# VITA-Group/Open-L2O

Measured on AMD Instinct MI355X. Metric: unroll-steps/sec (batch x params x T), L2O-DM on Quadratic d=128, higher is better.
Workload: dtype f32

## Files before the change

open_l2o_amd/csrc/l2o_lstm_bx3.h:

```cpp
#pragma once
#include <type_traits>
#include "l2o_common.h"

namespace l2o {
namespace bx {

typedef unsigned u32x4 __attribute__((ext_vector_type(4)));
typedef float f32x2 __attribute__((ext_vector_type(2)));
typedef __bf16 bf16x2 __attribute__((ext_vector_type(2)));
typedef __bf16 bf16x8 __attribute__((ext_vector_type(8)));

constexpr int kChL1H = 0, kChL2A = 1, kChL2B = 2, kChL1X = 3;
constexpr int kFragWords = 256;
constexpr int kPack = 4;
constexpr int kProducts = 6;
__host__ __device__ constexpr bool packed_default(int pre) { return pre != L2O_PRE_FC_ELU; }
__host__ __device__ constexpr int frags(bool pk) { return pk ? kPack : 3; }
__host__ __device__ constexpr int chunk_mfmas(bool pk) { return (pk ? kPack : kProducts) * kNT; }

__host__ __device__ constexpr int nchunks(int pre) { return pre == L2O_PRE_FC_ELU ? 4 : 3; }
__host__ __device__ constexpr int base(int pre) { return wp_rows(pre) * 64; }
__host__ __device__ constexpr int packed_words(int pre) { return nchunks(pre) * kNT * kPack * kFragWords; }
__host__ __device__ constexpr int level_words(int pre) { return nchunks(pre) * kNT * 3 * kFragWords; }
__host__ __device__ constexpr int frag_off(int pre, bool pk, int ch, int t, int j) {
// ... 176 lines not shown
        w.win1[t] = *reinterpret_cast<const f32x4*>(wp + win_off(PRE) + (kNT + t) * 256 + lane * 4);
    }
    w.wl[t] = p[(wp_row_wl(PRE) + t) * 64];
    if (PRE == L2O_PRE_FC_ELU) {
      w.fcw0[t] = p[(wp_row_fc(PRE) + t) * 64];
      w.fcw1[t] = p[(wp_row_fc(PRE) + kNT + t) * 64];
      w.fcb[t] = p[(wp_row_fc(PRE) + 2 * kNT + t) * 64];
    }
  }
  w.bl = p[wp_row_bl(PRE) * 64];
}

__device__ __forceinline__ f32x4 mfma_bf(u32x4 a, u32x4 b, f32x4 c) {
#ifdef L2O_ABLATE_MFMA
  c[0] = __builtin_fmaf(__uint_as_float(a[0]), __uint_as_float(b[0]), c[0]);
  return c;
#endif
  return __builtin_amdgcn_mfma_f32_16x16x32_bf16(__builtin_bit_cast(bf16x8, a), __builtin_bit_cast(bf16x8, b), c, 0,
                                                  0, 0);
}

template <int LAYER, class W, bool PIN = true>
__device__ __forceinline__ void preload_bias(const W& w, f32x4 (&acc)[kNT]) {
#pragma unroll
  for (int t = 0; t < kNT; ++t) acc[t] = w.bias[(LAYER * kNT + t) * 4];
  if constexpr (PIN) {
#pragma unroll
    for (int t = 0; t < kNT; ++t) asm volatile("" : "+v"(acc[t]));
  }
}

template <int PRE, int CH, int LO, int HI, bool ZERO, bool PK, class W>
__device__ __forceinline__ void issue_pipelined(const W& w, const BOp<PK>& b, f32x4 (&acc)[kNT]) {
  static_assert(PK && W::kLdsFrags, "issue_pipelined: the packed LDS-resident fragments");
  constexpr int DEP = W::kFragDepth;
  u32x4 f[DEP];
  static_for<0, DEP>([&](auto ic) {
    constexpr int i = decltype(ic)::value;
    if constexpr (LO + i < HI) {
      constexpr int n = LO + i;
      f[i] = w.lfr[((CH * kNT + n % kNT) * kPack + n / kNT) * 64];
    }
  });
  __builtin_amdgcn_sched_group_barrier(0x100, (HI - LO) < DEP ? (HI - LO) : DEP, 0);
  static_for<LO, HI>([&](auto nc) {
    constexpr int n = decltype(nc)::value;
    constexpr int p = n / kNT, t = n % kNT, slot = (n - LO) % DEP;
    acc[t] = mfma_bf(f[slot], b.m[p], acc[t]);
    if constexpr (n + DEP < HI) {
      constexpr int m = n + DEP;
      f[slot] = w.lfr[((CH * kNT + m % kNT) * kPack + m / kNT) * 64];
    }
    __builtin_amdgcn_sched_group_barrier(0x008, 1, 0);
    __builtin_amdgcn_sched_group_barrier(0x100, 1, 0);
  });
}

template <int PRE, int CH, int LO, int HI, bool ZERO, bool PK, class W>
__device__ __forceinline__ void issue(const W& w, const BOp<PK>& b, f32x4 (&acc)[kNT]) {
  if constexpr (W::kLdsFrags && W::kFragDepth > 0) {
    issue_pipelined<PRE, CH, LO, HI, ZERO, PK, W>(w, b, acc);
    return;
  }
  static_for<LO, HI>([&](auto nc) {
    constexpr int n = decltype(nc)::value;
    constexpr int p = n / kNT, t = n % kNT;
    if constexpr (W::kLdsFrags) {
      static_assert(PK, "LDS-resident fragments: the packed form");
#ifdef L2O_LDS_ABL_NOFRAG
      acc[t] = mfma_bf(b.m[(p + 1) % kPack], b.m[p], acc[t]);
#else
      acc[t] = mfma_bf(w.lfr[((CH * kNT + t) * kPack + p) * 64], b.m[p], acc[t]);
#endif
      if constexpr (W::kFragFence > 0) {
        if ((n - LO) % W::kFragFence == W::kFragFence - 1) __builtin_amdgcn_sched_barrier(0);
      }
    } else if constexpr (PK) acc[t] = mfma_bf(w.a[CH][t][p], b.m[p], acc[t]);
    else if constexpr (CH == W::kLdsChunk) acc[t] = mfma_bf(w.lch[(t * 3 + prod_w(p)) * 64], b.m[prod_x(p)], acc[t]);
    else acc[t] = mfma_bf(w.a[CH][t][prod_w(p)], b.m[prod_x(p)], acc[t]);
  });
}

template <int T0>
__device__ __forceinline__ void gates_pair(const f32x4 (&acc)[kNT], float (&c)[kNT], float (&h)[kNT]) {
  constexpr int T1 = T0 + 1;
  constexpr float k2 = 2.0f * 1.4426950408889634f;
  const f32x2 one = mk2(1.0f, 1.0f);
  const f32x2 e_i = mk2(fast_exp2(acc[T0][0]), fast_exp2(acc[T1][0]));
  const f32x2 E_j = mk2(fast_exp2(-__builtin_fabsf(acc[T0][1])), fast_exp2(-__builtin_fabsf(acc[T1][1])));
  const f32x2 e_f = mk2(fast_exp2(acc[T0][2]), fast_exp2(acc[T1][2]));
  const f32x2 e_o = mk2(fast_exp2(acc[T0][3]), fast_exp2(acc[T1][3]));
  const f32x2 dij = (one + e_i) * (one + E_j);
  const f32x2 df = one + e_f;
  const f32x2 ij = mk2(fast_rcp(dij.x), fast_rcp(dij.y));
  const f32x2 rf = mk2(fast_rcp(df.x), fast_rcp(df.y));
  f32x2 tj = (one - E_j) * ij;
  tj = mk2(__builtin_copysignf(tj.x, acc[T0][1]), __builtin_copysignf(tj.y, acc[T1][1]));
  const f32x2 cn = __builtin_elementwise_fma(rf, mk2(c[T0], c[T1]), tj);
  const f32x2 ca = cn * mk2(k2, k2);
  const f32x2 E_c = mk2(fast_exp2(-__builtin_fabsf(ca.x)), fast_exp2(-__builtin_fabsf(ca.y)));
  const f32x2 dro = (one + E_c) * (one + e_o);
  const f32x2 ro = mk2(fast_rcp(dro.x), fast_rcp(dro.y));
  const f32x2 hh = (one - E_c) * ro;
  c[T0] = cn.x; c[T1] = cn.y;
  h[T0] = __builtin_copysignf(hh.x, cn.x);
  h[T1] = __builtin_copysignf(hh.y, cn.y);
}

__device__ __forceinline__ void gates5(const f32x4 (&acc)[kNT], float (&c)[kNT], float (&h)[kNT]) {
#ifdef L2O_ABLATE_TRANS
#pragma unroll
  for (int t = 0; t < kNT; ++t) {
    c[t] = (acc[t][2] * 0.25f + 0.75f) * c[t] + (acc[t][0] * 0.25f + 0.5f) * (acc[t][1] * 0.5f);
    h[t] = (c[t] * 0.5f) * (acc[t][3] * 0.25f + 0.5f);
  }
  return;
#endif
#ifdef L2O_ABLATE_GATES
#pragma unroll
  for (int t = 0; t < kNT; ++t) { c[t] = acc[t][2] + acc[t][0]; h[t] = acc[t][1] + acc[t][3]; }
  return;
#endif
  gates_pair<0>(acc, c, h);
  gates_pair<2>(acc, c, h);
  constexpr float k2 = 2.0f * 1.4426950408889634f;
  const float e_i = fast_exp2(acc[4][0]), E_j = fast_exp2(-__builtin_fabsf(acc[4][1]));
  const float e_f = fast_exp2(acc[4][2]), e_o = fast_exp2(acc[4][3]);
  const float ij = fast_rcp((1.0f + e_i) * (1.0f + E_j)), rf = fast_rcp(1.0f + e_f);
  const float cn = __builtin_fmaf(rf, c[4], __builtin_copysignf((1.0f - E_j) * ij, acc[4][1]));
  const float E_c = fast_exp2(-__builtin_fabsf(cn * k2));
  const float ro = fast_rcp((1.0f + E_c) * (1.0f + e_o));
  c[4] = cn;
  h[4] = __builtin_copysignf((1.0f - E_c) * ro, cn);
}

__device__ __forceinline__ void gates5_scalar(const f32x4 (&acc)[kNT], float (&c)[kNT], float (&h)[kNT]) {
  constexpr float k2 = 2.0f * 1.4426950408889634f;
  float e_i[kNT], E_j[kNT], e_f[kNT], e_o[kNT], ij[kNT], rf[kNT], cn[kNT], E_c[kNT], ro[kNT];
#pragma unroll
  for (int t = 0; t < kNT; ++t) e_i[t] = fast_exp2(acc[t][0]);
#pragma unroll
  for (int t = 0; t < kNT; ++t) E_j[t] = fast_exp2(-__builtin_fabsf(acc[t][1]));
#pragma unroll
  for (int t = 0; t < kNT; ++t) e_f[t] = fast_exp2(acc[t][2]);
#pragma unroll
  for (int t = 0; t < kNT; ++t) e_o[t] = fast_exp2(acc[t][3]);
#pragma unroll
  for (int t = 0; t < kNT; ++t) ij[t] = fast_rcp((1.0f + e_i[t]) * (1.0f + E_j[t]));
#pragma unroll
  for (int t = 0; t < kNT; ++t) rf[t] = fast_rcp(1.0f + e_f[t]);
#pragma unroll
  for (int t = 0; t < kNT; ++t)
    cn[t] = __builtin_fmaf(rf[t], c[t], __builtin_copysignf((1.0f - E_j[t]) * ij[t], acc[t][1]));
#pragma unroll
  for (int t = 0; t < kNT; ++t) E_c[t] = fast_exp2(-__builtin_fabsf(cn[t] * k2));
#pragma unroll
  for (int t = 0; t < kNT; ++t) ro[t] = fast_rcp((1.0f + E_c[t]) * (1.0f + e_o[t]));
#pragma unroll
  for (int t = 0; t < kNT; ++t) {
    c[t] = cn[t];
    h[t] = __builtin_copysignf((1.0f - E_c[t]) * ro[t], cn[t]);
  }
}

struct NoShadow { __device__ __forceinline__ void operator()() const {} };
template <int PRE, bool NEXT, bool PK, class Shadow = NoShadow, bool REARM = true, class W = NetWB<PRE, PK>, bool SR = false>
__device__ __forceinline__ float finish(const W& w, TileState& s, BOp<PK>& b1, BOp<PK>& b2,
                                        f32x4 (&acc1)[kNT], f32x4 (&acc2)[kNT], float in0, float in1, unsigned one,
                                        int q, PhaseClock& pc, Shadow&& shadow = Shadow()) {
  constexpr int kN = chunk_mfmas(PK);
  static_assert(!SR || (PK && !NEXT && !W::kLdsFrags), "finish: the scalar-residual split is k_unroll_pair's");
  if constexpr (PRE == L2O_PRE_FC_ELU) {
    float fc[kNT];
#pragma unroll
    for (int t = 0; t < kNT; ++t)
      fc[t] = eluf_(__builtin_fmaf(w.fcw1[t], in1, __builtin_fmaf(w.fcw0[t], in0, w.fcb[t])));
    BOp<PK> bf;
    split5<PK>(fc, 0u, bf);
    issue<PRE, kChL1X, 0, kN, false>(w, bf, acc1);
  } else if constexpr (W::kLdsWin) {
#pragma unroll
    for (int t = 0; t < kNT; ++t) {
      acc1[t] += w.lwin[t * 64] * in0;
      if (PRE == L2O_PRE_LOGSIGN) acc1[t] += w.lwin[(kNT + t) * 64] * in1;
    }
  } else {
#pragma unroll
    for (int t = 0; t < kNT; ++t) {
      acc1[t] += w.win0[t] * in0;
      if (PRE == L2O_PRE_LOGSIGN) acc1[t] += w.win1[t] * in1;
    }
  }
  pc.drain(acc1);
  pc.mark(5);
  gates5(acc1, s.c1, s.h1);
#ifndef L2O_FINISH_PINNED_LDSFRAGS
#define L2O_FINISH_PINNED_LDSFRAGS 0
#endif
  constexpr bool kPinBias = !W::kLdsFrags || L2O_FINISH_PINNED_LDSFRAGS;
  if (REARM || NEXT) preload_bias<0, W, kPinBias>(w, acc1);
  pc.mark(6);
  split5<PK, SR>(s.h1, one, b1);
  issue<PRE, kChL2A, 0, kN, false>(w, b1, acc2);
  if constexpr (!std::is_same<typename std::decay<Shadow>::type, NoShadow>::value) {
    shadow();
#ifndef L2O_SHADOW_VALU_PER_MFMA
#define L2O_SHADOW_VALU_PER_MFMA 3
#endif
#pragma unroll
    for (int i = 0; i < kN; ++i) {
      __builtin_amdgcn_sched_group_barrier(0x008, 1, 0);
      __builtin_amdgcn_sched_group_barrier(0x002, L2O_SHADOW_VALU_PER_MFMA, 0);
    }
  }
  pc.mark(7);
  pc.drain(acc2);
  pc.mark(10);
  __builtin_amdgcn_sched_barrier(0);
  if (NEXT) {
#ifndef L2O_NEXT_VALU_PER_MFMA
#define L2O_NEXT_VALU_PER_MFMA 3
#endif
    issue<PRE, kChL1H, 0, kN, true>(w, b1, acc1);
    gates5_scalar(acc2, s.c2, s.h2);
#pragma unroll
    for (int i = 0; i < kN; ++i) {
      __builtin_amdgcn_sched_group_barrier(0x008, 1, 0);
      __builtin_amdgcn_sched_group_barrier(0x402, L2O_NEXT_VALU_PER_MFMA, 0);
    }
  } else {
    gates5(acc2, s.c2, s.h2);
  }
  __builtin_amdgcn_sched_barrier(0);
  if (REARM) preload_bias<1, W, kPinBias>(w, acc2);
  pc.mark(8);
  if (NEXT) split5<PK>(s.h2, one, b2);
  float d0 = s.h2[0] * w.wl[0], d1 = s.h2[1] * w.wl[1];
  d0 = __builtin_fmaf(s.h2[2], w.wl[2], d0);
  d1 = __builtin_fmaf(s.h2[3], w.wl[3], d1);
  d0 = __builtin_fmaf(s.h2[4], w.wl[4], d0);
  const float d = quad_q_sum(d0 + d1);
  return d + w.bl;
}

template <int PRE, bool PK, class W>
__device__ __forceinline__ float tile_step_w(const W& w, TileState& s, float in0, float in1, int q) {
  const unsigned one = bias_one<PK>(q);
  constexpr int kN = chunk_mfmas(PK);
  BOp<PK> b1, b2;
  f32x4 acc1[kNT], acc2[kNT];
#ifdef L2O_TILE_STEP_PINNED
  preload_bias<1>(w, acc2);
  preload_bias<0>(w, acc1);
  split5<PK>(s.h2, one, b2);
#else
  preload_bias<1, W, false>(w, acc2);
  preload_bias<0, W, false>(w, acc1);
  split5<PK>(s.h2, one, b2);
  __builtin_amdgcn_sched_group_barrier(0x100, 2 * kNT, 0);
  __builtin_amdgcn_sched_group_barrier(0x002, 32, 0);
#endif
  issue<PRE, kChL2B, 0, kN, true>(w, b2, acc2);
  split5<PK>(s.h1, one, b1);
  issue<PRE, kChL1H, 0, kN, true>(w, b1, acc1);
  PhaseClock pc;
  return finish<PRE, false, PK, NoShadow, false, W>(w, s, b1, b2, acc1, acc2, in0, in1, one, q, pc);
}
template <int PRE, bool PK>
__device__ __forceinline__ float tile_step(const NetWB<PRE, PK>& w, TileState& s, float in0, float in1, int q) {
  return tile_step_w<PRE, PK, NetWB<PRE, PK>>(w, s, in0, in1, q);
}

template <int PRE, int CH, class W>
__device__ __forceinline__ void issue2(const W& w, const BOp<true>& ba, const BOp<true>& bb, f32x4 (&acca)[kNT], f32x4 (&accb)[kNT]) {
  static_assert(W::kLdsFrags, "issue2: the LDS-resident packed fragments");
  static_for<0, chunk_mfmas(true)>([&](auto nc) {
    constexpr int n = decltype(nc)::value;
    constexpr int p = n / kNT, t = n % kNT;
// ... 106 lines not shown

template <int PRE, bool PK, class WT, bool SR = false>
struct LstmCoreRegs {
  static constexpr int kTotal = bx::chunk_mfmas(PK), kHalf = kTotal / 2;
  WT w;
  bx::BOp<PK> b1, b2;
  unsigned one;
  __device__ __forceinline__ void load(const float* __restrict__ wpack, int lane) { bx::load_netw<PRE, true, PK, WT::kLdsChunk>(w, wpack, lane); }
  static constexpr int kStageFrags = WT::kLdsChunk < 0 ? WT::NCH * kNT * bx::frags(PK) : 0;
  static constexpr int kStageOff = bx::frag_off(PRE, PK, 0, 0, 0);
  __device__ __forceinline__ void load_small(const float* __restrict__ wpack, int lane) { bx::load_netw<PRE, false, PK>(w, wpack, lane); }
  __device__ __forceinline__ void read_stage(const float4* stage, int lane) {
#pragma unroll
    for (int ch = 0; ch < WT::NCH; ++ch)
#pragma unroll
      for (int t = 0; t < kNT; ++t)
#pragma unroll
        for (int j = 0; j < bx::frags(PK); ++j)
          w.a[ch][t][j] = __builtin_bit_cast(bx::u32x4, stage[((ch * kNT + t) * bx::frags(PK) + j) * 64 + lane]);
  }
  static constexpr int kBiasFloats = bx::kBiasWords;
  __device__ __forceinline__ void stage_bias(float* lds, const float* __restrict__ wpack, int tid, int nthreads, int q) {
    bx::stage_bias(lds, wpack, PRE, tid, nthreads);
    bx::set_bias(w, lds, q);
  }
  template <int NTHREADS>
  __device__ __forceinline__ void fetch_bias(float (&v)[(bx::kBiasWords + NTHREADS - 1) / NTHREADS], const float* __restrict__ wpack, int tid) {
#pragma unroll
    for (int k = 0; k < (bx::kBiasWords + NTHREADS - 1) / NTHREADS; ++k) {
      const int i = tid + k * NTHREADS;
      v[k] = wpack[bx::bias_off(PRE) + (i < bx::kBiasWords ? i : bx::kBiasWords - 1)];
    }
  }
  template <int NTHREADS>
  __device__ __forceinline__ void put_bias(float* lds, const float (&v)[(bx::kBiasWords + NTHREADS - 1) / NTHREADS], int tid, int q) {
#pragma unroll
    for (int k = 0; k < (bx::kBiasWords + NTHREADS - 1) / NTHREADS; ++k) {
      const int i = tid + k * NTHREADS;
      if (i < bx::kBiasWords) lds[i] = v[k];
    }
    bx::set_bias(w, lds, q);
  }
  __device__ __forceinline__ void pin() {
#ifndef L2O_NO_AGPR_PIN
#pragma unroll
    for (int ch = 0; ch < WT::NCH; ++ch)
#pragma unroll
      for (int t = 0; t < kNT; ++t)
#pragma unroll
        for (int j = 0; j < bx::frags(PK); ++j)
          if (ch != WT::kLdsChunk) asm volatile("" : "+a"(w.a[ch][t][j]));
#endif
  }
  __device__ __forceinline__ void init(const TileState& s, int q) {
    one = bx::bias_one<PK>(q);
    bx::split5<PK>(s.h1, one, b1);
    bx::split5<PK>(s.h2, one, b2);
  }
  __device__ __forceinline__ void preload(f32x4 (&acc1)[kNT], f32x4 (&acc2)[kNT]) {
    bx::preload_bias<0>(w, acc1);
    bx::preload_bias<1>(w, acc2);
  }
  __device__ __forceinline__ void preload_unpinned(f32x4 (&acc1)[kNT], f32x4 (&acc2)[kNT]) {
    bx::preload_bias<0, WT, false>(w, acc1);
    bx::preload_bias<1, WT, false>(w, acc2);
  }
  f32x4 bias1r[kNT], bias2r[kNT];
  __device__ __forceinline__ void hold_bias() {
    bx::preload_bias<0>(w, bias1r);
    bx::preload_bias<1>(w, bias2r);
  }
  __device__ __forceinline__ void arm(f32x4 (&acc1)[kNT], f32x4 (&acc2)[kNT]) const {
#pragma unroll
    for (int t = 0; t < kNT; ++t) { acc1[t] = bias1r[t]; acc2[t] = bias2r[t]; }
  }
  template <int LO, int HI>
  __device__ __forceinline__ void issue_l1_prev(const TileState&, f32x4 (&acc1)[kNT]) {
    bx::issue<PRE, bx::kChL1H, LO, HI, true>(w, b1, acc1);
  }
  template <int LO, int HI>
  __device__ __forceinline__ void issue_l2_prev(const TileState&, f32x4 (&acc2)[kNT]) {
    bx::issue<PRE, bx::kChL2B, LO, HI, true>(w, b2, acc2);
  }
  template <bool NEXT, class Shadow = bx::NoShadow, bool REARM = true>
  __device__ __forceinline__ float finish(TileState& s, f32x4 (&acc1)[kNT], f32x4 (&acc2)[kNT], float in0, float in1,
                                          int q, PhaseClock& pc, Shadow&& shadow = Shadow()) {
    return bx::finish<PRE, NEXT, PK, Shadow, REARM, WT, SR>(w, s, b1, b2, acc1, acc2, in0, in1, one, q, pc, static_cast<Shadow&&>(shadow));
  }
  __device__ __forceinline__ void refresh(const TileState& s) { bx::split5<PK, SR>(s.h2, one, b2); }
};
template <int PRE, bool PK>
struct LstmCore<PRE, true, PK> : LstmCoreRegs<PRE, PK, bx::NetWB<PRE, PK>> {};
#ifndef L2O_PAIR_SPLIT_SCALAR
#define L2O_PAIR_SPLIT_SCALAR 1
#endif
template <int PRE, bool BX, bool FAST, bool PK = bx::packed_default(PRE)>
struct LstmCorePair : LstmCore<PRE, BX, PK> {};
template <int PRE>
struct LstmCorePair<PRE, true, true, true> : LstmCoreRegs<PRE, true, bx::NetWB<PRE, true>, L2O_PAIR_SPLIT_SCALAR != 0> {};
template <int PRE, int KIND, int CH, bool HIST, bool EXACT, bool FAST>
constexpr bool kPairBiasRegs =
    !HIST && !EXACT &&
    (FAST || !(PRE == L2O_PRE_LOGSIGN && (KIND == L2O_PROB_RASTRIGIN || KIND == L2O_PROB_SQUARE_COS) && CH == 8));
template <int PRE, int LDSCH>
struct LstmCoreHyb : LstmCoreRegs<PRE, false, bx::NetWBH<PRE, LDSCH>> {
  static constexpr int kChunkFloats = bx::NetWBH<PRE, LDSCH>::kChunkFloats;
  __device__ __forceinline__ void stage_chunk(float* lds, const float* __restrict__ wpack, int tid, int nthreads, int lane) {
    const unsigned* wu = reinterpret_cast<const unsigned*>(wpack);
    bx::u32x4* dst = reinterpret_cast<bx::u32x4*>(lds);
    for (int i = tid; i < kChunkFloats / 4; i += nthreads) {
      const int f = i >> 6, l = i & 63;
      dst[i] = *reinterpret_cast<const bx::u32x4*>(wu + bx::frag_off(PRE, false, LDSCH, f / 3, f % 3) + l * 4);
    }
    this->w.lch = reinterpret_cast<const __attribute__((address_space(3))) bx::u32x4*>(
                      (const __attribute__((address_space(3))) float*)lds) + lane;
  }
};

namespace bx {
#ifndef L2O_CU8_FRAG_FENCE
#define L2O_CU8_FRAG_FENCE 0
#endif
#ifndef L2O_CU8_LDS_WIN
#define L2O_CU8_LDS_WIN 1
#endif
template <int PRE, int DEPTH = L2O_CU8_FRAG_DEPTH>
struct NetWBLF : NetWBL<PRE> {
  static constexpr int kFragFence = L2O_CU8_FRAG_FENCE;
  static constexpr int kFragDepth = DEPTH;
  static constexpr bool kLdsWin = L2O_CU8_LDS_WIN && PRE != L2O_PRE_FC_ELU;
  const __attribute__((address_space(3))) f32x4* lwin;
  static constexpr int kWinFloats = PRE == L2O_PRE_FC_ELU ? 0 : (PRE == L2O_PRE_LOGSIGN ? 2 : 1) * kNT * 256;
};
template <int PRE, int DEPTH>
__device__ __forceinline__ void stage_win(NetWBLF<PRE, DEPTH>& w, float* lds, const float* __restrict__ wp, int tid, int nthreads, int lane) {
  if constexpr (NetWBLF<PRE, DEPTH>::kLdsWin) {
    const f32x4* src = reinterpret_cast<const f32x4*>(wp + win_off(PRE));
    f32x4* dst = reinterpret_cast<f32x4*>(lds);
    for (int i = tid; i < NetWBLF<PRE, DEPTH>::kWinFloats / 4; i += nthreads) dst[i] = src[i];
    w.lwin = reinterpret_cast<const __attribute__((address_space(3))) f32x4*>((const __attribute__((address_space(3))) float*)lds) + lane;
  }
}
}

template <int PRE, class WT = bx::NetWBL<PRE>>
struct LstmCoreLds {
  static constexpr int kTotal = bx::chunk_mfmas(true), kHalf = kTotal / 2;
  static constexpr int kFragWords = bx::packed_words(PRE);
  WT w;
  bx::BOp<true> b1, b2;
  unsigned one;
  __device__ __forceinline__ void load(const float* __restrict__ wpack, int lane) { bx::load_netw<PRE, false, true, -1, WT::kLdsWin>(w, wpack, lane); }
  __device__ __forceinline__ void stage_frags(float* lds, const float* __restrict__ wpack, int tid, int nthreads, int lane) {
    const bx::u32x4* src = reinterpret_cast<const bx::u32x4*>(wpack + bx::base(PRE));
    bx::u32x4* dst = reinterpret_cast<bx::u32x4*>(lds);
    for (int i = tid; i < kFragWords / 4; i += nthreads) dst[i] = src[i];
    w.lfr = reinterpret_cast<const __attribute__((address_space(3))) bx::u32x4*>(
                (const __attribute__((address_space(3))) float*)lds) + lane;
  }
  static constexpr int kBiasFloats = bx::kBiasWords;
  __device__ __forceinline__ void stage_bias(float* lds, const float* __restrict__ wpack, int tid, int nthreads, int q) {
    bx::stage_bias(lds, wpack, PRE, tid, nthreads);
    bx::set_bias(w, lds, q);
  }
  __device__ __forceinline__ void pin() {}
  __device__ __forceinline__ void init(const TileState& s, int q) {
    one = bx::bias_one<true>(q);
    bx::split5<true>(s.h1, one, b1);
    bx::split5<true>(s.h2, one, b2);
  }
  __device__ __forceinline__ void preload(f32x4 (&acc1)[kNT], f32x4 (&acc2)[kNT]) {
    bx::preload_bias<0>(w, acc1);
    bx::preload_bias<1>(w, acc2);
  }
  __device__ __forceinline__ void preload_unpinned(f32x4 (&acc1)[kNT], f32x4 (&acc2)[kNT]) {
    bx::preload_bias<0, WT, false>(w, acc1);
    bx::preload_bias<1, WT, false>(w, acc2);
  }
  template <int LO, int HI>
  __device__ __forceinline__ void issue_l1_prev(const TileState&, f32x4 (&acc1)[kNT]) {
    bx::issue<PRE, bx::kChL1H, LO, HI, true>(w, b1, acc1);
  }
  template <int LO, int HI>
  __device__ __forceinline__ void issue_l2_prev(const TileState&, f32x4 (&acc2)[kNT]) {
    bx::issue<PRE, bx::kChL2B, LO, HI, true>(w, b2, acc2);
  }
// ... 10 lines not shown
```

open_l2o_amd/csrc/l2o_unroll_pair.h:

```cpp
#pragma once
#include "l2o_lstm_bx3.h"
#include "l2o_params.h"

struct PairWs {
  unsigned status;
  unsigned seq;
  unsigned fault;
  unsigned pad0;
  long long ticks;
  long long ticks_total;
  unsigned pad[8];
  long long phases[16];
};
static_assert(sizeof(PairWs) == 64 + 128, "workspace header layout (include/l2o_abi.h)");

struct UnrollPairArgs {
  UnrollArgs u;
  PairWs* ws;
  unsigned long long* xbuf;
  float* fx_half;
  unsigned use_salt;
  unsigned plain_stores;
  int b0, nb;
  unsigned fast_load;
// ... 134 lines not shown
      for (int k = 0; k < 4; ++k) {
        const int row = 16 * m + 4 * gq + k;
        e[k] = (row < M && col < D) ? Wb[(size_t)row * D + col] : 0.0f;
      }
      wt[m] = make_float4(e[0], e[1], e[2], e[3]);
    }
  }
  constexpr bool kPk = L2O_GEMV_PK != 0;
  l2o::f32x4 wrq[2][NWH], wtq[CH];
#pragma unroll
  for (int m = 0; m < NWH; ++m) { wrq[0][m] = as_quad(wr[0][m]); wrq[1][m] = as_quad(wr[1][m]); }
#pragma unroll
  for (int m = 0; m < CH; ++m) wtq[m] = as_quad(wt[m]);
  const int myrow = (2 * wv + (gq & 1)) * kTile + gr;
  const float myy = (gq < 2 && myrow < M) ? pp.y[(size_t)b * M + myrow] : 0.0f;
  const bool row_counted = gq < 2 && (half == 0 ? (myrow < NC) : (myrow >= NC));

  using Core = LstmCorePair<PRE, !EXACT, false>;
  Core core;
  core.load(a.np.wpack, lane);
  core.pin();
  __shared__ __attribute__((aligned(16))) float bias_s[Core::kBiasFloats];
  core.stage_bias(bias_s, a.np.wpack, tid, blockDim.x, q);
  L2O_LAUNCH_MARK(1);
  const int j = tile_in_prob * kTile + c;
  const bool live = j < D;
  const size_t idx = (size_t)b * D + j;
  const int tpp = (D + kTile - 1) / kTile;
  const bool tile_real = tile_in_prob < tpp;
  TileState s;
  float* st_tile = a.st + ((size_t)b * tpp + (tile_real ? tile_in_prob : 0)) * kStateFloatsPerTile;
  if (tile_real && !a.zero_state) load_tile_state(s, st_tile, lane);
  else {
#pragma unroll
    for (int t = 0; t < kNT; ++t) s.h1[t] = s.c1[t] = s.h2[t] = s.c2[t] = 0.0f;
  }
  float xv = live ? (a.x_in ? a.x_in : a.x)[idx] : 0.0f;
  const float sc = (live && pp.x_scale) ? pp.x_scale[idx] : 1.0f;
  float cj = 0.0f;
  constexpr bool kCos = KIND == L2O_PROB_RASTRIGIN || KIND == L2O_PROB_SQUARE_COS;
  if (kCos) cj = live ? pp.C[idx] : 0.0f;
  float mv = 0.0f, vv = 0.0f;
  if (PRE == L2O_PRE_FC_ELU && !a.zero_state) { mv = live ? a.m[idx] : 0.0f; vv = live ? a.v[idx] : 0.0f; }
  float p1h = a.p1_hi, p1l = a.p1_lo, p2h = a.p2_hi, p2l = a.p2_lo;
  constexpr bool kSq = KIND == L2O_PROB_QUADRATIC || KIND == L2O_PROB_SQUARE_COS;
  const float coef = kSq ? 1.0f : 0.5f;
  const float cg = (KIND == L2O_PROB_QUADRATIC ? 2.0f : 1.0f) * pp.inv_bg;
  const float kTwoPi = pp.twopi;
  const float* xsq = xs + 4 * gq;
  const float* rsq = rs + 4 * gq;
  unsigned long long* mine = pa.xbuf + ((size_t)bl * 2 + half) * 2 * SQ;
  const unsigned long long* theirs = pa.xbuf + ((size_t)bl * 2 + (half ^ 1)) * 2 * SQ;
  bool dead = false;
  if (pa.ws->fault != 0) {
    dead = true;
    if (tid == 0) atomicExch(&pa.ws->status, 1u);
  }
  L2O_LAUNCH_MARK_LANDED(2);
  __shared__ __attribute__((aligned(16))) int same_xcd_s4[4];
  int& same_xcd_s = same_xcd_s4[0];
  if (tid == 0) {
    unsigned my_xcc;
    asm volatile("s_getreg_b32 %0, hwreg(HW_REG_XCC_ID)" : "=s"(my_xcc));
    my_xcc &= 0xfu;
    const unsigned kHsTag = 0x80000000u | salt | 0xffffu;
    __hip_atomic_store(mine + SQ, ((unsigned long long)kHsTag << 32) | my_xcc, __ATOMIC_RELAXED, __HIP_MEMORY_SCOPE_AGENT);
    unsigned long long g = 0;
    int spins = 0;
    bool ok = true;
#pragma nounroll
    for (;;) {
      g = __hip_atomic_load(theirs + SQ, __ATOMIC_RELAXED, __HIP_MEMORY_SCOPE_AGENT);
      if ((unsigned)(g >> 32) == kHsTag) break;
      if (dead || ++spins > (1 << 20)) { ok = false; break; }
      __builtin_amdgcn_s_sleep(1);
    }
    same_xcd_s = ok && pa.plain_stores && ((unsigned)g & 0xfu) == my_xcc;
  }
  __syncthreads();
  const bool same_xcd = same_xcd_s != 0;
  L2O_LAUNCH_MARK(3);

  constexpr bool kBiasRegs = kPairBiasRegs<PRE, KIND, CH, HIST, EXACT, false>;
#define L2O_PAIR_FX_PTR 0
#include "l2o_unroll_pair_loop.h"
#undef L2O_PAIR_FX_PTR
}

template <int PRE, int KIND, int CH, bool HIST, bool EXACT>
__device__ __forceinline__ void unroll_pair_body(const UnrollPairArgs& pa) {
  const long long kernel_t0 = __builtin_readcyclecounter();
#ifdef L2O_PROFILE_PHASES
  unsigned launch_marks[8] = {0, 0, 0, 0, 0, 0, 0, 0};
#endif
  constexpr int SQ = 16 * CH;
  constexpr int NWH = CH / 2;
  constexpr int NC = 16 * NWH;
  __shared__ __attribute__((aligned(16))) float xs[NC];
  __shared__ __attribute__((aligned(16))) float rs[SQ];
  const UnrollArgs& a = pa.u;
  const ProbParams& pp = a.pp;
  const int D = pp.D, M = pp.M;
  const int tid = threadIdx.x, lane = tid & 63, wv = tid >> 6;
  const int c = lane & 15, q = lane >> 4;
  const int bid = blockIdx.x;
  const int half = (bid >> 3) & 1;
  const int bl = ((bid >> 4) << 3) | (bid & 7);
  if (bl >= pa.nb) return;
  const int b = pa.b0 + bl;
  const int tile_in_prob = half * NWH + wv;
  const int gq = q, gr = c;

  using Core = LstmCorePair<PRE, !EXACT, true>;
  constexpr bool kStage = Core::kStageFrags > 0 && NWH >= 2;
  __shared__ float4 frag_stage[kStage ? Core::kStageFrags * 64 : 1];
  static_assert(sizeof(frag_stage) + sizeof(float) * (NC + SQ + Core::kBiasFloats + 4) <= 64 * 1024, "static LDS");
  if constexpr (kStage) {
    const int wvs = __builtin_amdgcn_readfirstlane(wv);
    const float* src = a.np.wpack + Core::kStageOff + lane * 4;
#pragma unroll
    for (int f = 0; f < (Core::kStageFrags + NWH - 1) / NWH; ++f) {
      const int fr = NWH * f + wvs;
      if (Core::kStageFrags % NWH == 0 || fr < Core::kStageFrags)
        __builtin_amdgcn_global_load_lds((gbl_void*)(src + fr * bx::kFragWords), (lds_void*)(frag_stage + fr * 64), 16, 0, 0);
    }
  }

  const float* Wb = pp.W + (pp.w_shared ? (size_t)0 : (size_t)b * M * D);
  const int col0 = half * NC;
  float4 wr[2][NWH], wt[CH];
  if (pa.fast_load && M == SQ && D == SQ && (reinterpret_cast<size_t>(pp.W) & 15) == 0) {
    const float4* Wq = reinterpret_cast<const float4*>(Wb + (size_t)(2 * wv * kTile + gr) * SQ + col0 + 4 * gq);
#pragma unroll
    for (int p = 0; p < 2; ++p)
#pragma unroll
      for (int m = 0; m < NWH; ++m) wr[p][m] = Wq[(p * kTile * SQ + 16 * m) / 4];
    const float* Wc = Wb + (size_t)(4 * gq) * SQ + col0 + wv * kTile + gr;
#pragma unroll
    for (int m = 0; m < CH; ++m)
      wt[m] = make_float4(Wc[(16 * m + 0) * SQ], Wc[(16 * m + 1) * SQ], Wc[(16 * m + 2) * SQ], Wc[(16 * m + 3) * SQ]);
  } else {
#pragma unroll
    for (int p = 0; p < 2; ++p) {
      const int row = (2 * wv + p) * kTile + gr;
#pragma unroll
      for (int m = 0; m < NWH; ++m) {
        float e[4];
#pragma unroll
        for (int k = 0; k < 4; ++k) {
          const int col = col0 + 16 * m + 4 * gq + k;
          e[k] = (row < M && col < D) ? Wb[(size_t)row * D + col] : 0.0f;
        }
        wr[p][m] = make_float4(e[0], e[1], e[2], e[3]);
      }
    }
    const int col = col0 + wv * kTile + gr;
#pragma unroll
    for (int m = 0; m < CH; ++m) {
      float e[4];
#pragma unroll
      for (int k = 0; k < 4; ++k) {
        const int row = 16 * m + 4 * gq + k;
        e[k] = (row < M && col < D) ? Wb[(size_t)row * D + col] : 0.0f;
      }
      wt[m] = make_float4(e[0], e[1], e[2], e[3]);
    }
// ... 34 lines not shown
    core.load(a.np.wpack, lane);
  __builtin_amdgcn_sched_barrier(0);
  L2O_LAUNCH_MARK(1);

  if constexpr (kStage) {
    L2O_LAUNCH_MARK_LANDED(2);
    asm volatile("s_waitcnt vmcnt(0)" ::: "memory");
  }
  const unsigned seq_w = __builtin_amdgcn_readfirstlane(seq_v), fault_w = __builtin_amdgcn_readfirstlane(fault_v);
  const unsigned salt = pa.use_salt ? ((seq_w + 1u) & 0x7fffu) << 16 : 0u;
  unsigned long long* mine = pa.xbuf + ((size_t)bl * 2 + half) * 2 * SQ;
  const unsigned long long* theirs = pa.xbuf + ((size_t)bl * 2 + (half ^ 1)) * 2 * SQ;
  const unsigned kHsTag = 0x80000000u | salt | 0xffffu;
  unsigned my_xcc = 0;
  if (tid == 0) {
    asm volatile("s_getreg_b32 %0, hwreg(HW_REG_XCC_ID)" : "=s"(my_xcc));
    my_xcc &= 0xfu;
    __hip_atomic_store(mine + SQ, ((unsigned long long)kHsTag << 32) | my_xcc, __ATOMIC_RELAXED, __HIP_MEMORY_SCOPE_AGENT);
  }
  L2O_LAUNCH_MARK(0);
  __builtin_amdgcn_sched_barrier(0);
  __shared__ __attribute__((aligned(16))) float bias_s[Core::kBiasFloats];
  if constexpr (kStage) core.template put_bias<64 * NWH>(bias_s, bias_ld, tid, q);
  else core.stage_bias(bias_s, a.np.wpack, tid, 64 * NWH, q);
  if constexpr (kStage) {
    asm volatile("s_waitcnt lgkmcnt(0)" ::: "memory");
    __builtin_amdgcn_s_barrier();
    asm volatile("" ::: "memory");
    core.read_stage(frag_stage, lane);
    __builtin_amdgcn_sched_barrier(0);
  } else
    core.pin();
  constexpr bool kPk = L2O_GEMV_PK != 0;
  l2o::f32x4 wrq[2][NWH], wtq[CH];
#pragma unroll
  for (int m = 0; m < NWH; ++m) { wrq[0][m] = as_quad(wr[0][m]); wrq[1][m] = as_quad(wr[1][m]); }
#pragma unroll
  for (int m = 0; m < CH; ++m) wtq[m] = as_quad(wt[m]);
  TileState s;
  unpack_tile_state(s, st_ld);
  if (!(tile_real && !a.zero_state)) {
#pragma unroll
    for (int t = 0; t < kNT; ++t) s.h1[t] = s.c1[t] = s.h2[t] = s.c2[t] = 0.0f;
  }
  const float myy = (gq < 2 && myrow < M) ? y_ld : 0.0f;
  float xv = live ? x_ld : 0.0f;
  const float sc = live ? sc_ld : 1.0f;
  const float cj = live ? cj_ld : 0.0f;
  float mv = live ? m_ld : 0.0f, vv = live ? v_ld : 0.0f;
  float p1h = a.p1_hi, p1l = a.p1_lo, p2h = a.p2_hi, p2l = a.p2_lo;
  constexpr bool kSq = KIND == L2O_PROB_QUADRATIC || KIND == L2O_PROB_SQUARE_COS;
  const float coef = kSq ? 1.0f : 0.5f;
  const float cg = (KIND == L2O_PROB_QUADRATIC ? 2.0f : 1.0f) * pp.inv_bg;
  const float kTwoPi = pp.twopi;
  const float* xsq = xs + 4 * gq;
  const float* rsq = rs + 4 * gq;
  bool dead = false;
  if (fault_w != 0) {
    dead = true;
    if (tid == 0) atomicExch(&pa.ws->status, 1u);
  }
  if constexpr (!kStage) L2O_LAUNCH_MARK_LANDED(2);
  __shared__ __attribute__((aligned(16))) int same_xcd_s4[4];
  int& same_xcd_s = same_xcd_s4[0];
  if (tid == 0) {
    unsigned long long g = 0;
    int spins = 0;
    bool ok = true;
#pragma nounroll
    for (;;) {
      g = __hip_atomic_load(theirs + SQ, __ATOMIC_RELAXED, __HIP_MEMORY_SCOPE_AGENT);
      if ((unsigned)(g >> 32) == kHsTag) break;
      if (dead || ++spins > (1 << 20)) { ok = false; break; }
      __builtin_amdgcn_s_sleep(1);
    }
    same_xcd_s = ok && pa.plain_stores && ((unsigned)g & 0xfu) == my_xcc;
  }
  __syncthreads();
  const bool same_xcd = same_xcd_s != 0;
  if constexpr (kStage) core.pin();
  L2O_LAUNCH_MARK(3);

  constexpr bool kBiasRegs = kPairBiasRegs<PRE, KIND, CH, HIST, EXACT, true>;
#define L2O_PAIR_FX_PTR 1
#include "l2o_unroll_pair_loop.h"
#undef L2O_PAIR_FX_PTR
}

template <int PRE, int KIND, int CH, bool HIST, bool EXACT = false, bool FAST = false>
__global__ __launch_bounds__(256) void k_unroll_pair(UnrollPairArgs pa) {
  if constexpr (FAST) unroll_pair_body<PRE, KIND, CH, HIST, EXACT>(pa);
  else unroll_pair_body_gather<PRE, KIND, CH, HIST, EXACT>(pa);
}
```

open_l2o_amd/csrc/l2o_unroll_pair_step_head.h:

```cpp
    const float xsv = xv * sc;
    const unsigned tag = salt | ((unsigned)t + 1u);
    const int par = t & 1;
    pc.mark(0);
    if (HIST || L2O_PAIR_LDS_BARRIERS) lds_barrier(); else __syncthreads();
    pc.mark(2);
    float part;
    {
      float4 r0 = {0.f, 0.f, 0.f, 0.f}, r1 = {0.f, 0.f, 0.f, 0.f};
      Acc4pk r0p = {{0.f, 0.f}, {0.f, 0.f}}, r1p = {{0.f, 0.f}, {0.f, 0.f}};
      l2o::f32x4 x4v[NWH];
      lds_load_f4<NWH>(x4v, xsq);
      core.refresh(s);
      __builtin_amdgcn_sched_group_barrier(0x100, NWH, 0);
      __builtin_amdgcn_sched_group_barrier(0x002, 48, 0);
#pragma unroll
      for (int m = 0; m < NWH; ++m) {
        if (kPk) { dot4pk(wrq[0][m], x4v[m], r0p); dot4pk(wrq[1][m], x4v[m], r1p); }
        else { dot4v(wr[0][m], x4v[m], r0); dot4v(wr[1][m], x4v[m], r1); }
      }
      const float h0 = kPk ? hsum4pk(r0p) : hsum4(r0), h1 = kPk ? hsum4pk(r1p) : hsum4(r1);
      const u32x2 sw = __builtin_amdgcn_permlane16_swap(__float_as_uint(h0), __float_as_uint(h1), false, false);
      part = xor32_add(__uint_as_float(sw[0]) + __uint_as_float(sw[1]));
    }
    {
      unsigned long long* const pub = mine + par * SQ + myrow;
      if (__builtin_expect(!same_xcd, 0)) {
        asm volatile("");
        if (gq < 2) __hip_atomic_store(pub, pack_granule(part, tag), __ATOMIC_RELAXED, __HIP_MEMORY_SCOPE_AGENT);
      }
      if (pub_plain) __hip_atomic_store(pub, pack_granule(part, tag), __ATOMIC_RELAXED, __HIP_MEMORY_SCOPE_WORKGROUP);
    }
    l2o::SinCos trig = {0.0f, 1.0f};
    if (kCos) trig = l2o::sincos_f(kTwoPi * xsv);
    pc.mark(3);
#ifndef L2O_PAIR_POLL_AT
#define L2O_PAIR_POLL_AT 20
#endif
    constexpr int kPollAt = L2O_PAIR_POLL_AT < Core::kTotal ? L2O_PAIR_POLL_AT : Core::kTotal;
    constexpr int kPollAt1 = L2O_PAIR_POLL_AT > Core::kTotal ? L2O_PAIR_POLL_AT - Core::kTotal : 0;
    core.template issue_l2_prev<0, kPollAt>(s, acc2);
    if (kPollAt1 > 0) core.template issue_l1_prev<0, kPollAt1>(s, acc1);
    const unsigned long long* src = theirs + par * SQ + (gq < 2 ? myrow : 0);
    unsigned long long g = 0;
    const unsigned poll_tag = poll_salt | ((unsigned)t + 1u);
    __builtin_amdgcn_sched_barrier(0);
#ifndef L2O_ABLATE_EXCHANGE
    if (gq < 2) g = __hip_atomic_load(src, __ATOMIC_RELAXED, __HIP_MEMORY_SCOPE_AGENT);
#endif
    __builtin_amdgcn_sched_barrier(0);
    if (kPollAt < Core::kTotal) core.template issue_l2_prev<kPollAt, Core::kTotal>(s, acc2);
    core.template issue_l1_prev<kPollAt1, Core::kTotal>(s, acc1);
    float contrib = 0.0f;
    if (gq < 2) {
      int spins = 0;
#ifdef L2O_ABLATE_EXCHANGE
      const bool wait = false;
#else
      const bool wait = (unsigned)(g >> 32) != poll_tag;
#endif
      if (__builtin_expect(__builtin_amdgcn_ballot_w64(wait) != 0, 0)) {
        asm volatile("");
        bool timed_out = false;
        if (poll_salt != salt) g = 0;
        else if (wait) {
#pragma nounroll
          for (;;) {
            g = __hip_atomic_load(src, __ATOMIC_RELAXED, __HIP_MEMORY_SCOPE_AGENT);
            if ((unsigned)(g >> 32) == tag) break;
            if (++spins > (1 << 20)) { timed_out = true; atomicExch(&pa.ws->status, 1u); break; }
#ifndef L2O_POLL_NOSLEEP
            __builtin_amdgcn_s_sleep(1);
#endif
          }
        }
        if (__builtin_amdgcn_ballot_w64(timed_out) != 0) poll_salt = salt | 0x80000000u;
      }
      const float r = (part + __uint_as_float((unsigned)g)) - myy;
      rs[myrow] = r;
      if (row_counted) contrib = coef * r * r;
    }
    if (live && q == 0) {
      if (KIND == L2O_PROB_LASSO) contrib += pp.l1 * __builtin_fabsf(xsv);
      if (kCos) contrib += pp.alpha - pp.alpha * cj * trig.c;
    }
    if (HIST && t < a.T && tile_real)
      store_tile_state(s, a.hist_st + ((size_t)t * pp.B_local * tpp + (size_t)b * tpp + tile_in_prob) *
                                          kStateFloatsPerTile, lane);
    pc.mark(1);
    if (HIST || L2O_PAIR_LDS_BARRIERS) lds_barrier(); else __syncthreads();
    pc.mark(4);
    l2o::f32x4 rv4v[CH];
    lds_load_f4<CH>(rv4v, rsq);
    {
      const float fw = wave_sum64(contrib);
      __builtin_amdgcn_sched_group_barrier(0x100, CH, 0);
      __builtin_amdgcn_sched_group_barrier(0x002, 24, 0);
#if L2O_PAIR_FX_PTR
      *fxp = fw;
      fxp += fx_stride;
#else
      pa.fx_half[((size_t)t * pa.nb + bl) * (2 * NWH) + half * NWH + wv] = fw;
#endif
    }
```

open_l2o_amd/csrc/l2o_unroll_pair_step_tail.h:

```cpp
    constexpr bool kPkG = L2O_GEMV_PK_G != 0;
    float4 gacc4 = {0.f, 0.f, 0.f, 0.f};
    Acc4pk gaccp = {{0.f, 0.f}, {0.f, 0.f}};
#pragma unroll
    for (int m = 0; m < CH; ++m) {
      if (kPkG) dot4pk(wtq[m], rv4v[m], gaccp);
      else dot4v(wt[m], rv4v[m], gacc4);
    }
    float gv = quad_q_sum(kPkG ? hsum4pk(gaccp) : hsum4(gacc4));
    if (KIND == L2O_PROB_SQUARE_COS) gv *= 2.0f;
    if (KIND == L2O_PROB_LASSO) gv += pp.l1 * (xsv > 0.f ? 1.f : (xsv < 0.f ? -1.f : 0.f));
    if (kCos) gv += kTwoPi * pp.alpha * cj * trig.s;
    gv = live ? gv * cg * sc : 0.0f;
    if (HIST && live && q == 0) {
      if (t < a.T) a.hist_g[(size_t)t * hist_n + idx] = gv;
      else a.hist_gfinal[idx] = gv;
    }
    if (HIST && t == a.T) break;

    float in0, in1;
    if (PRE == L2O_PRE_FC_ELU) {
      rnnprop_inputs(gv, mv, vv, a.np.beta1, a.np.beta2, a.np.omb1, a.np.omb2, 1.0f - p1h, 1.0f - p2h, in0, in1);
      if (HIST && live && q == 0) { a.hist_m[(size_t)t * hist_n + idx] = mv; a.hist_v[(size_t)t * hist_n + idx] = vv; }
      if (!live) { in0 = 0.0f; in1 = 0.0f; }
      {
        float hi = p1h * a.np.beta1, er = __builtin_fmaf(p1h, a.np.beta1, -hi);
        float lo = __builtin_fmaf(p1l, a.np.beta1, er), sum = hi + lo;
        p1l = lo - (sum - hi); p1h = sum;
        hi = p2h * a.np.beta2; er = __builtin_fmaf(p2h, a.np.beta2, -hi);
        lo = __builtin_fmaf(p2l, a.np.beta2, er); sum = hi + lo;
        p2l = lo - (sum - hi); p2h = sum;
      }
    } else {
      preprocess_grad<PRE>(gv, a.np.k_inv_ln2, a.np.exp_k, in0, in1);
    }
    float d = core.template finish<false, bx::NoShadow, false>(s, acc1, acc2, in0, in1, q, pc);
    if (__builtin_expect(a.np.tanh_output != 0, 0)) {
      asm volatile("");
      d = tanhf_(d);
    }
    xv = __builtin_fmaf(d, a.np.scale, xv);
    __builtin_amdgcn_sched_barrier(0);
    xs[wv * kTile + c] = live ? xv * sc : 0.0f;
    __builtin_amdgcn_sched_barrier(0);
    if constexpr (kBiasRegs) core.arm(acc1, acc2);
    else core.preload_unpinned(acc1, acc2);
    __builtin_amdgcn_sched_barrier(0);
    pc.mark(9);
```

Baseline: 10.78 billion.

## Defer tail of layer-2 recurrent MFMAs to overlap gate exps and reduction

Splits the layer-2 previous-h (L2B) MFMA chunk so the last 15 MFMAs are not issued in the step head. Seven of them are interleaved with the wave-sum/fx store after the exchange barrier, and the remaining eight run inside finish alongside the layer-1 gate exponentials, which are separated out into gates5_exps/gates5_rest. The head schedule is also rewritten to interleave MFMA with VALU and to place the cross-wave poll load at a fixed earlier position (10 instead of 20). The aim is to hide the transcendental and reduction latency under matrix work on the serial critical path, at the cost of longer live ranges for the b2 operands and acc2.

```diff
diff --git a/open_l2o_amd/csrc/l2o_lstm_bx3.h b/open_l2o_amd/csrc/l2o_lstm_bx3.h
--- a/open_l2o_amd/csrc/l2o_lstm_bx3.h
+++ b/open_l2o_amd/csrc/l2o_lstm_bx3.h
@@ -282,14 +282,11 @@
 }
 
 template <int T0>
-__device__ __forceinline__ void gates_pair(const f32x4 (&acc)[kNT], float (&c)[kNT], float (&h)[kNT]) {
+__device__ __forceinline__ void gates_pair_e(const f32x4 (&acc)[kNT], float (&c)[kNT], float (&h)[kNT], const f32x2 e_i,
+                                             const f32x2 E_j, const f32x2 e_f, const f32x2 e_o) {
   constexpr int T1 = T0 + 1;
   constexpr float k2 = 2.0f * 1.4426950408889634f;
   const f32x2 one = mk2(1.0f, 1.0f);
-  const f32x2 e_i = mk2(fast_exp2(acc[T0][0]), fast_exp2(acc[T1][0]));
-  const f32x2 E_j = mk2(fast_exp2(-__builtin_fabsf(acc[T0][1])), fast_exp2(-__builtin_fabsf(acc[T1][1])));
-  const f32x2 e_f = mk2(fast_exp2(acc[T0][2]), fast_exp2(acc[T1][2]));
-  const f32x2 e_o = mk2(fast_exp2(acc[T0][3]), fast_exp2(acc[T1][3]));
   const f32x2 dij = (one + e_i) * (one + E_j);
   const f32x2 df = one + e_f;
   const f32x2 ij = mk2(fast_rcp(dij.x), fast_rcp(dij.y));
@@ -306,6 +303,15 @@
   h[T0] = __builtin_copysignf(hh.x, cn.x);
   h[T1] = __builtin_copysignf(hh.y, cn.y);
 }
+template <int T0>
+__device__ __forceinline__ void gates_pair(const f32x4 (&acc)[kNT], float (&c)[kNT], float (&h)[kNT]) {
+  constexpr int T1 = T0 + 1;
+  const f32x2 e_i = mk2(fast_exp2(acc[T0][0]), fast_exp2(acc[T1][0]));
+  const f32x2 E_j = mk2(fast_exp2(-__builtin_fabsf(acc[T0][1])), fast_exp2(-__builtin_fabsf(acc[T1][1])));
+  const f32x2 e_f = mk2(fast_exp2(acc[T0][2]), fast_exp2(acc[T1][2]));
+  const f32x2 e_o = mk2(fast_exp2(acc[T0][3]), fast_exp2(acc[T1][3]));
+  gates_pair_e<T0>(acc, c, h, e_i, E_j, e_f, e_o);
+}
 
 __device__ __forceinline__ void gates5(const f32x4 (&acc)[kNT], float (&c)[kNT], float (&h)[kNT]) {
 #ifdef L2O_ABLATE_TRANS
@@ -363,13 +369,35 @@
   }
 }
 
+struct GateExps { f32x4 e[kNT]; };
+__device__ __forceinline__ void gates5_exps(const f32x4 (&acc)[kNT], GateExps& g) {
+  static_for<0, 4 * kNT>([&](auto nc) {
+    constexpr int k = decltype(nc)::value / kNT, t = decltype(nc)::value % kNT;
+    g.e[t][k] = fast_exp2(k == 1 ? -__builtin_fabsf(acc[t][1]) : acc[t][k]);
+  });
+}
+__device__ __forceinline__ void gates5_rest(const f32x4 (&acc)[kNT], const GateExps& g, float (&c)[kNT], float (&h)[kNT]) {
+  gates_pair_e<0>(acc, c, h, mk2(g.e[0][0], g.e[1][0]), mk2(g.e[0][1], g.e[1][1]), mk2(g.e[0][2], g.e[1][2]), mk2(g.e[0][3], g.e[1][3]));
+  gates_pair_e<2>(acc, c, h, mk2(g.e[2][0], g.e[3][0]), mk2(g.e[2][1], g.e[3][1]), mk2(g.e[2][2], g.e[3][2]), mk2(g.e[2][3], g.e[3][3]));
+  constexpr float k2 = 2.0f * 1.4426950408889634f;
+  const float e_i = g.e[4][0], E_j = g.e[4][1], e_f = g.e[4][2], e_o = g.e[4][3];
+  const float ij = fast_rcp((1.0f + e_i) * (1.0f + E_j)), rf = fast_rcp(1.0f + e_f);
+  const float cn = __builtin_fmaf(rf, c[4], __builtin_copysignf((1.0f - E_j) * ij, acc[4][1]));
+  const float E_c = fast_exp2(-__builtin_fabsf(cn * k2));
+  const float ro = fast_rcp((1.0f + E_c) * (1.0f + e_o));
+  c[4] = cn;
+  h[4] = __builtin_copysignf((1.0f - E_c) * ro, cn);
+}
+
 struct NoShadow { __device__ __forceinline__ void operator()() const {} };
-template <int PRE, bool NEXT, bool PK, class Shadow = NoShadow, bool REARM = true, class W = NetWB<PRE, PK>, bool SR = false>
+template <int PRE, bool NEXT, bool PK, class Shadow = NoShadow, bool REARM = true, class W = NetWB<PRE, PK>, bool SR = false,
+          int L2B_LATE = 0>
 __device__ __forceinline__ float finish(const W& w, TileState& s, BOp<PK>& b1, BOp<PK>& b2,
                                         f32x4 (&acc1)[kNT], f32x4 (&acc2)[kNT], float in0, float in1, unsigned one,
                                         int q, PhaseClock& pc, Shadow&& shadow = Shadow()) {
   constexpr int kN = chunk_mfmas(PK);
   static_assert(!SR || (PK && !NEXT && !W::kLdsFrags), "finish: the scalar-residual split is k_unroll_pair's");
+  static_assert(L2B_LATE == 0 || (PK && !NEXT && !W::kLdsFrags && L2B_LATE <= kN), "finish: the late part of chunk L2B is k_unroll_pair's");
   if constexpr (PRE == L2O_PRE_FC_ELU) {
     float fc[kNT];
 #pragma unroll
@@ -393,7 +421,20 @@
   }
   pc.drain(acc1);
   pc.mark(5);
-  gates5(acc1, s.c1, s.h1);
+  if constexpr (L2B_LATE > 0) {
+    __builtin_amdgcn_sched_barrier(0);
+    issue<PRE, kChL2B, kN - L2B_LATE, kN, true>(w, b2, acc2);
+    GateExps ge;
+    gates5_exps(acc1, ge);
+#pragma unroll
+    for (int i = 0; i < L2B_LATE; ++i) {
+      __builtin_amdgcn_sched_group_barrier(0x008, 1, 0);
+      __builtin_amdgcn_sched_group_barrier(0x400, 1, 0);
+    }
+    __builtin_amdgcn_sched_barrier(0);
+    gates5_rest(acc1, ge, s.c1, s.h1);
+  } else
+    gates5(acc1, s.c1, s.h1);
 #ifndef L2O_FINISH_PINNED_LDSFRAGS
 #define L2O_FINISH_PINNED_LDSFRAGS 0
 #endif
@@ -666,12 +707,16 @@
   __device__ __forceinline__ void issue_l2_prev(const TileState&, f32x4 (&acc2)[kNT]) {
     bx::issue<PRE, bx::kChL2B, LO, HI, true>(w, b2, acc2);
   }
-  template <bool NEXT, class Shadow = bx::NoShadow, bool REARM = true>
+  template <bool NEXT, class Shadow = bx::NoShadow, bool REARM = true, int L2B_LATE = 0>
   __device__ __forceinline__ float finish(TileState& s, f32x4 (&acc1)[kNT], f32x4 (&acc2)[kNT], float in0, float in1,
                                           int q, PhaseClock& pc, Shadow&& shadow = Shadow()) {
-    return bx::finish<PRE, NEXT, PK, Shadow, REARM, WT, SR>(w, s, b1, b2, acc1, acc2, in0, in1, one, q, pc, static_cast<Shadow&&>(shadow));
+    return bx::finish<PRE, NEXT, PK, Shadow, REARM, WT, SR, L2B_LATE>(w, s, b1, b2, acc1, acc2, in0, in1, one, q, pc, static_cast<Shadow&&>(shadow));
   }
   __device__ __forceinline__ void refresh(const TileState& s) { bx::split5<PK, SR>(s.h2, one, b2); }
+  __device__ __forceinline__ void hold_b2() {
+#pragma unroll
+    for (int j = 0; j < bx::kPack; ++j) asm volatile("" : "+v"(b2.m[j]));
+  }
 };
 template <int PRE, bool PK>
 struct LstmCore<PRE, true, PK> : LstmCoreRegs<PRE, PK, bx::NetWB<PRE, PK>> {};
@@ -686,6 +731,11 @@
 constexpr bool kPairBiasRegs =
     !HIST && !EXACT &&
     (FAST || !(PRE == L2O_PRE_LOGSIGN && (KIND == L2O_PROB_RASTRIGIN || KIND == L2O_PROB_SQUARE_COS) && CH == 8));
+template <int PRE, int KIND, int CH, bool HIST, bool EXACT, bool FAST>
+constexpr int kPairL2bLate =
+    (FAST && !HIST && !EXACT && bx::packed_default(PRE) && !(PRE == L2O_PRE_LOGSIGN && CH == 8)) ? 15 : 0;
+constexpr int kPairL2bB2 = 7;
+constexpr int kPairPollAtLate = 10;
 template <int PRE, int LDSCH>
 struct LstmCoreHyb : LstmCoreRegs<PRE, false, bx::NetWBH<PRE, LDSCH>> {
   static constexpr int kChunkFloats = bx::NetWBH<PRE, LDSCH>::kChunkFloats;
diff --git a/open_l2o_amd/csrc/l2o_unroll_pair.h b/open_l2o_amd/csrc/l2o_unroll_pair.h
--- a/open_l2o_amd/csrc/l2o_unroll_pair.h
+++ b/open_l2o_amd/csrc/l2o_unroll_pair.h
@@ -240,6 +240,7 @@
   L2O_LAUNCH_MARK(3);
 
   constexpr bool kBiasRegs = kPairBiasRegs<PRE, KIND, CH, HIST, EXACT, false>;
+  constexpr int kL2bLate = kPairL2bLate<PRE, KIND, CH, HIST, EXACT, false>;
 #define L2O_PAIR_FX_PTR 0
 #include "l2o_unroll_pair_loop.h"
 #undef L2O_PAIR_FX_PTR
@@ -440,6 +441,7 @@
   L2O_LAUNCH_MARK(3);
 
   constexpr bool kBiasRegs = kPairBiasRegs<PRE, KIND, CH, HIST, EXACT, true>;
+  constexpr int kL2bLate = kPairL2bLate<PRE, KIND, CH, HIST, EXACT, true>;
 #define L2O_PAIR_FX_PTR 1
 #include "l2o_unroll_pair_loop.h"
 #undef L2O_PAIR_FX_PTR
diff --git a/open_l2o_amd/csrc/l2o_unroll_pair_step_head.h b/open_l2o_amd/csrc/l2o_unroll_pair_step_head.h
--- a/open_l2o_amd/csrc/l2o_unroll_pair_step_head.h
+++ b/open_l2o_amd/csrc/l2o_unroll_pair_step_head.h
@@ -10,7 +10,7 @@
       Acc4pk r0p = {{0.f, 0.f}, {0.f, 0.f}}, r1p = {{0.f, 0.f}, {0.f, 0.f}};
       l2o::f32x4 x4v[NWH];
       lds_load_f4<NWH>(x4v, xsq);
-      core.refresh(s);
+      if constexpr (kL2bLate == 0) core.refresh(s);
       __builtin_amdgcn_sched_group_barrier(0x100, NWH, 0);
       __builtin_amdgcn_sched_group_barrier(0x002, 48, 0);
 #pragma unroll
@@ -36,20 +36,42 @@
 #ifndef L2O_PAIR_POLL_AT
 #define L2O_PAIR_POLL_AT 20
 #endif
-    constexpr int kPollAt = L2O_PAIR_POLL_AT < Core::kTotal ? L2O_PAIR_POLL_AT : Core::kTotal;
-    constexpr int kPollAt1 = L2O_PAIR_POLL_AT > Core::kTotal ? L2O_PAIR_POLL_AT - Core::kTotal : 0;
-    core.template issue_l2_prev<0, kPollAt>(s, acc2);
-    if (kPollAt1 > 0) core.template issue_l1_prev<0, kPollAt1>(s, acc1);
+    constexpr int kL2bB2 = kL2bLate > 0 ? kPairL2bB2 : 0;
+    constexpr int kWinL2 = Core::kTotal - kL2bLate;
+    constexpr int kPollN = kL2bLate > 0 ? kPairPollAtLate : L2O_PAIR_POLL_AT;
+    constexpr int kPollAt = kPollN < kWinL2 ? kPollN : kWinL2;
+    constexpr int kPollAt1 = kPollN > kWinL2 ? (kPollN - kWinL2 < Core::kTotal ? kPollN - kWinL2 : Core::kTotal) : 0;
+    if constexpr (kL2bLate > 0) {
+      core.refresh(s);
+      core.template issue_l2_prev<0, kWinL2>(s, acc2);
+      core.template issue_l1_prev<0, Core::kTotal>(s, acc1);
+    } else {
+      core.template issue_l2_prev<0, kPollAt>(s, acc2);
+      if (kPollAt1 > 0) core.template issue_l1_prev<0, kPollAt1>(s, acc1);
+    }
     const unsigned long long* src = theirs + par * SQ + (gq < 2 ? myrow : 0);
     unsigned long long g = 0;
     const unsigned poll_tag = poll_salt | ((unsigned)t + 1u);
-    __builtin_amdgcn_sched_barrier(0);
+    if constexpr (kL2bLate > 0) {
 #ifndef L2O_ABLATE_EXCHANGE
-    if (gq < 2) g = __hip_atomic_load(src, __ATOMIC_RELAXED, __HIP_MEMORY_SCOPE_AGENT);
+      g = __hip_atomic_load(src, __ATOMIC_RELAXED, __HIP_MEMORY_SCOPE_AGENT);
 #endif
-    __builtin_amdgcn_sched_barrier(0);
-    if (kPollAt < Core::kTotal) core.template issue_l2_prev<kPollAt, Core::kTotal>(s, acc2);
-    core.template issue_l1_prev<kPollAt1, Core::kTotal>(s, acc1);
+      core.hold_b2();
+#pragma unroll
+      for (int i = 0; i < kWinL2 + Core::kTotal; ++i) {
+        if (i == kPollN) __builtin_amdgcn_sched_group_barrier(0x020, 1, 0);
+        __builtin_amdgcn_sched_group_barrier(0x008, 1, 0);
+        __builtin_amdgcn_sched_group_barrier(0x002, 2, 0);
+      }
+    } else {
+      __builtin_amdgcn_sched_barrier(0);
+#ifndef L2O_ABLATE_EXCHANGE
+      if (gq < 2) g = __hip_atomic_load(src, __ATOMIC_RELAXED, __HIP_MEMORY_SCOPE_AGENT);
+#endif
+      __builtin_amdgcn_sched_barrier(0);
+      if (kPollAt < kWinL2) core.template issue_l2_prev<kPollAt, kWinL2>(s, acc2);
+      core.template issue_l1_prev<kPollAt1, Core::kTotal>(s, acc1);
+    }
     float contrib = 0.0f;
     if (gq < 2) {
       int spins = 0;
@@ -92,8 +114,16 @@
     l2o::f32x4 rv4v[CH];
     lds_load_f4<CH>(rv4v, rsq);
     {
+      if constexpr (kL2bB2 > 0) core.template issue_l2_prev<kWinL2, kWinL2 + kL2bB2>(s, acc2);
       const float fw = wave_sum64(contrib);
       __builtin_amdgcn_sched_group_barrier(0x100, CH, 0);
+      if constexpr (kL2bB2 > 0) {
+#pragma unroll
+        for (int i = 0; i < kL2bB2; ++i) {
+          __builtin_amdgcn_sched_group_barrier(0x008, 1, 0);
+          __builtin_amdgcn_sched_group_barrier(0x002, 2, 0);
+        }
+      } else
       __builtin_amdgcn_sched_group_barrier(0x002, 24, 0);
 #if L2O_PAIR_FX_PTR
       *fxp = fw;
@@ -101,4 +131,5 @@
 #else
       pa.fx_half[((size_t)t * pa.nb + bl) * (2 * NWH) + half * NWH + wv] = fw;
 #endif
+      if constexpr (kL2bB2 > 0) __builtin_amdgcn_sched_barrier(0);
     }
diff --git a/open_l2o_amd/csrc/l2o_unroll_pair_step_tail.h b/open_l2o_amd/csrc/l2o_unroll_pair_step_tail.h
--- a/open_l2o_amd/csrc/l2o_unroll_pair_step_tail.h
+++ b/open_l2o_amd/csrc/l2o_unroll_pair_step_tail.h
@@ -33,7 +33,9 @@
     } else {
       preprocess_grad<PRE>(gv, a.np.k_inv_ln2, a.np.exp_k, in0, in1);
     }
-    float d = core.template finish<false, bx::NoShadow, false>(s, acc1, acc2, in0, in1, q, pc);
+    float d;
+    if constexpr (kL2bLate > 0) d = core.template finish<false, bx::NoShadow, false, kL2bLate - kL2bB2>(s, acc1, acc2, in0, in1, q, pc);
+    else d = core.template finish<false, bx::NoShadow, false>(s, acc1, acc2, in0, in1, q, pc);
     if (__builtin_expect(a.np.tanh_output != 0, 0)) {
       asm volatile("");
       d = tanhf_(d);
```

Result: faster. 10.99 billion, median of 6 (+2.0%).
